# frgfm/Holocron

Measured on NVIDIA H100. Metric: images/sec RepVGG-A0 224^2 bf16 train, higher is better.
Workload: dtype bf16

## Files before the change

### holocron_b200/csrc/bn_act.cu

```cuda
#include <cstdio>
#include <cstdlib>
#include <type_traits>
#include <utility>
#include "common.cuh"
#include "act.cuh"
#include "slab.cuh"

namespace {

using namespace hb;

constexpr int kThreads = kSlabThreads;
constexpr int kMaxBranches = 3;

struct Branches {
  const __nv_bfloat16* u[kMaxBranches];
  int n;
};

__device__ __forceinline__ void fold_stat_partials(const SlabGeo& g, const float* red, int C, float* parts) {
  fold_row_lanes<double, 2>(g, red, [&](int c, const double (&a)[2]) {
    *reinterpret_cast<float2*>(parts + ((size_t)blockIdx.x * C + c) * 2) = make_float2((float)a[0], (float)a[1]);
  });
}
// ... 139 lines not shown
__global__ void bn_eval_affine_kernel(const float* gamma, const float* beta, const float* rmean, const float* rvar,
                                      float eps, int C, int C_logical, float* scale, float* shift, float* mean,
                                      float* rstd) {
  const int c = blockIdx.x * blockDim.x + threadIdx.x;
  if (c >= C) return;
  if (c >= C_logical) {
    scale[c] = 0.f; shift[c] = 0.f;
    if (mean) mean[c] = 0.f;
    if (rstd) rstd[c] = 0.f;
    return;
  }
  const float r = 1.f / sqrtf(rvar[c] + eps);
  const float sc = (gamma ? gamma[c] : 1.f) * r;
  scale[c] = sc;
  shift[c] = (beta ? beta[c] : 0.f) - rmean[c] * sc;
  if (mean) mean[c] = rmean[c];
  if (rstd) rstd[c] = r;
}

struct FwdParams {
  Branches br;
  const float* scale;
  const float* shift;
  const __nv_bfloat16* residual;
  __nv_bfloat16* out;
  int M, C, act;
  float slope;
  int res_after;
  float* out_stats;
};
using RawVec = Vec16<__nv_bfloat16>;

__device__ __forceinline__ void lds8(const float* p, float* f) {
  const float4 a = *reinterpret_cast<const float4*>(p);
  const float4 b = *reinterpret_cast<const float4*>(p + 4);
  f[0] = a.x; f[1] = a.y; f[2] = a.z; f[3] = a.w; f[4] = b.x; f[5] = b.y; f[6] = b.z; f[7] = b.w;
}

__host__ __device__ constexpr int ring_depth(int nt) { return nt <= 2 ? 7 : 3; }

__device__ __forceinline__ void cp_async16(uint32_t saddr, const void* g) {
  asm volatile("cp.async.cg.shared.global [%0], [%1], 16;" ::"r"(saddr), "l"(g) : "memory");
}
__device__ __forceinline__ void cp_async_commit() { asm volatile("cp.async.commit_group;" ::: "memory"); }
template <int N>
__device__ __forceinline__ void cp_async_wait() { asm volatile("cp.async.wait_group %0;" ::"n"(N) : "memory"); }
__device__ __forceinline__ RawVec lds16(uint32_t saddr) {
  RawVec r;
  asm volatile("ld.shared.v4.u32 {%0,%1,%2,%3}, [%4];" : "=r"(r.raw.x), "=r"(r.raw.y), "=r"(r.raw.z), "=r"(r.raw.w) : "r"(saddr));
  return r;
}
__device__ __forceinline__ uint32_t smem_addr(const void* p) { return (uint32_t)__cvta_generic_to_shared(p); }

template <int NT>
struct RowRing {
  static constexpr int kDepth = ring_depth(NT);
  static constexpr int kSlots = kDepth + 1;
  uint32_t base;
  size_t m0, stride, M;
  size_t col_off;
  int C;
  const __nv_bfloat16* src[NT > 0 ? NT : 1];
  __device__ __forceinline__ void init(uint8_t* smem, size_t m0_, size_t stride_, int M_, int C_, size_t col_off_) {
    base = smem_addr(smem) + threadIdx.x * 16;
    m0 = m0_; stride = stride_; M = (size_t)M_; col_off = col_off_; C = C_;
  }
  __device__ __forceinline__ uint32_t addr(int s, int t) const { return base + (uint32_t)((s * NT + t) * kThreads * 16); }
  __device__ __forceinline__ bool valid(size_t k) const { return m0 + k * stride < M; }
  __device__ __forceinline__ size_t off(size_t k) const { return (m0 + k * stride) * C + col_off; }
  __device__ __forceinline__ void issue(size_t k) const {
    if (valid(k)) {
      const int s = (int)(k % kSlots);
      const size_t o = off(k);
#pragma unroll
      for (int t = 0; t < NT; ++t)
        if (src[t]) cp_async16(addr(s, t), src[t] + o);
    }
    cp_async_commit();
  }
  __device__ __forceinline__ void prologue() const {
#pragma unroll
    for (int k = 0; k < kDepth; ++k) issue(k);
  }
  __device__ __forceinline__ void wait() const { cp_async_wait<kDepth - 1>(); }
};

template <int NB, bool kStats>
__global__ void __launch_bounds__(kThreads, 3) bn_act_fwd_kernel(FwdParams p, SlabGeo g) {
  extern __shared__ __align__(16) uint8_t ring_smem[];
  const auto [tx, ty, cg, active] = g.thread();
  float os[8], oq[8];
#pragma unroll
  for (int j = 0; j < 8; ++j) { os[j] = 0.f; oq[j] = 0.f; }
  __shared__ __align__(16) float k_sc[kMaxBranches][256];
  __shared__ __align__(16) float k_sh[256];
  {
    const int nch = g.cg_t * 8;
    for (int ch = threadIdx.x; ch < nch; ch += kThreads) {
      const int c = blockIdx.y * nch + ch;
      float shv = 0.f;
#pragma unroll
      for (int b = 0; b < NB; ++b) {
        k_sc[b][ch] = c < p.C ? p.scale[(size_t)b * p.C + c] : 0.f;
        shv += c < p.C ? p.shift[(size_t)b * p.C + c] : 0.f;
      }
      k_sh[ch] = shv;
    }
    __syncthreads();
  }
  if (!active && !kStats) return;
  if (active) {
    const bool has_res = p.residual != nullptr;
    RowRing<NB + 1> ring;
    ring.init(ring_smem, (size_t)blockIdx.x * g.rows_t + ty, (size_t)gridDim.x * g.rows_t, p.M, p.C, (size_t)cg * 8);
#pragma unroll
    for (int b = 0; b < NB; ++b) ring.src[b] = p.br.u[b];
    ring.src[NB] = p.residual;
    ring.prologue();
    for (size_t k = 0; ring.valid(k); ++k) {
      ring.wait();
      const int s = (int)(k % RowRing<NB + 1>::kSlots);
      RawVec u[NB > 0 ? NB : 1], r;
// ... 99 lines not shown
        const double mean = (double)p.mean[o], rstd = (double)p.rstd[o];
        const double mdzx = rstd * (p.sums[(size_t)(1 + b) * p.C + c] * invM - mean * mdz);
        const double cud = -(double)sc * rstd * mdzx;
        cu = (float)cud;
        c0 = (float)(-(double)sc * mdz - cud * mean);
      }
      k.cu[b][ch] = cu;
      k.c0[b][ch] = c0;
    }
    k.shift[ch] = sh;
  }
  __syncthreads();
}

template <int NB>
__device__ __forceinline__ void recompute_dz(const BwdParams& p, const SlabConsts& k, int ch0, const RawVec* uv,
                                             const RawVec& rv, const RawVec& dv, float (*u)[8], float* dz, float* dr) {
  float z[8];
  lds8(&k.shift[ch0], z);
#pragma unroll
  for (int b = 0; b < NB; ++b) {
    float sc[8];
    lds8(&k.scale[b][ch0], sc);
    unpack8(uv[b], u[b]);
#pragma unroll
    for (int j = 0; j < 8; ++j) z[j] = fmaf(sc[j], u[b][j], z[j]);
  }
  float d[8];
  unpack8(dv, d);
  if (p.residual && p.res_after) {
#pragma unroll
    for (int j = 0; j < 8; ++j) { dz[j] = d[j] * act_grad(p.act, z[j], p.slope); dr[j] = d[j]; }
    return;
  }
  if (p.residual) {
    float r[8];
    unpack8(rv, r);
    if (p.act == ACT_FRELU) {
#pragma unroll
      for (int j = 0; j < 8; ++j) {
        const float gate = z[j] > r[j] ? 1.f : (z[j] == r[j] ? 0.5f : 0.f);
        dz[j] = d[j] * gate;
        dr[j] = d[j] - dz[j];
      }
      return;
    }
#pragma unroll
    for (int j = 0; j < 8; ++j) z[j] += r[j];
  }
#pragma unroll
  for (int j = 0; j < 8; ++j) { dz[j] = d[j] * act_grad(p.act, z[j], p.slope); dr[j] = dz[j]; }
}

template <int NB>
__device__ __forceinline__ void init_bwd_ring(RowRing<NB + 2>& ring, const BwdParams& p, const SlabGeo& g, uint8_t* ring_smem,
                                              int ty, int cg) {
  ring.init(ring_smem, (size_t)blockIdx.x * g.rows_t + ty, (size_t)gridDim.x * g.rows_t, p.M, p.C, (size_t)cg * 8);
#pragma unroll
  for (int b = 0; b < NB; ++b) ring.src[b] = p.br.u[b];
  ring.src[NB] = (p.residual && !p.res_after) ? p.residual : nullptr;
  ring.src[NB + 1] = p.dout;
}

template <int NB>
__global__ void __launch_bounds__(kThreads, 2) bn_act_bwd_reduce_kernel(BwdParams p, SlabGeo g) {
  extern __shared__ __align__(16) uint8_t dyn_smem[];
  SlabConsts& k = *reinterpret_cast<SlabConsts*>(dyn_smem);
  float* red = reinterpret_cast<float*>(dyn_smem + sizeof(SlabConsts));
  uint8_t* ring_smem = dyn_smem + sizeof(SlabConsts) + kThreads * 8 * sizeof(float);
  load_slab_consts<NB>(k, p, g, false);
  const auto [tx, ty, cg, active] = g.thread();
  float acc[1 + NB][8];
#pragma unroll
  for (int i = 0; i < 1 + NB; ++i)
#pragma unroll
    for (int j = 0; j < 8; ++j) acc[i][j] = 0.f;
  if (active) {
    RowRing<NB + 2> ring;
    init_bwd_ring<NB>(ring, p, g, ring_smem, ty, cg);
    ring.prologue();
    for (size_t kk = 0; ring.valid(kk); ++kk) {
      ring.wait();
      const int s = (int)(kk % RowRing<NB + 2>::kSlots);
      RawVec uv[NB > 0 ? NB : 1], rv, dv;
#pragma unroll
      for (int b = 0; b < NB; ++b) uv[b] = lds16(ring.addr(s, b));
      if (ring.src[NB]) rv = lds16(ring.addr(s, NB));
      dv = lds16(ring.addr(s, NB + 1));
      ring.issue(kk + RowRing<NB + 2>::kDepth);
      float u[NB > 0 ? NB : 1][8], dz[8], dr[8];
      recompute_dz<NB>(p, k, tx * 8, uv, rv, dv, u, dz, dr);
#pragma unroll
      for (int j = 0; j < 8; ++j) acc[0][j] += dz[j];
#pragma unroll
      for (int b = 0; b < NB; ++b) {
#pragma unroll
        for (int j = 0; j < 8; ++j) acc[1 + b][j] = fmaf(dz[j], u[b][j], acc[1 + b][j]);
      }
    }
  }
#pragma unroll
  for (int i = 0; i < 1 + NB; ++i) {
    __syncthreads();
#pragma unroll
    for (int j = 0; j < 8; ++j) red[threadIdx.x * 8 + j] = acc[i][j];
    __syncthreads();
    fold_row_lanes<double, 1>(g, red, [&](int c, const double (&a)[1]) {
      p.part[((size_t)blockIdx.x * (1 + NB) + i) * p.C + c] = a[0];
    });
  }
}

template <int NB>
__global__ void __launch_bounds__(kThreads, 2) bn_act_bwd_apply_kernel(BwdParams p, SlabGeo g) {
  extern __shared__ __align__(16) uint8_t dyn_smem[];
  SlabConsts& k = *reinterpret_cast<SlabConsts*>(dyn_smem);
  uint8_t* ring_smem = dyn_smem + sizeof(SlabConsts);
  load_slab_consts<NB>(k, p, g, true);
  const auto [tx, ty, cg, active] = g.thread();
  if (!active) return;
  RowRing<NB + 2> ring;
  init_bwd_ring<NB>(ring, p, g, ring_smem, ty, cg);
  ring.prologue();
  for (size_t kk = 0; ring.valid(kk); ++kk) {
    ring.wait();
    const int s = (int)(kk % RowRing<NB + 2>::kSlots);
    RawVec uv[NB > 0 ? NB : 1], rv, dv;
#pragma unroll
    for (int b = 0; b < NB; ++b) uv[b] = lds16(ring.addr(s, b));
    if (ring.src[NB]) rv = lds16(ring.addr(s, NB));
    dv = lds16(ring.addr(s, NB + 1));
    ring.issue(kk + RowRing<NB + 2>::kDepth);
    const size_t off = ring.off(kk);
    float u[NB > 0 ? NB : 1][8], dz[8], dr[8];
    recompute_dz<NB>(p, k, tx * 8, uv, rv, dv, u, dz, dr);
    if (p.dres) store8(p.dres + off, dr);
#pragma unroll
    for (int b = 0; b < NB; ++b) {
      if (p.du[b]) {
        float sc[8], cu[8], c0[8], d[8];
        lds8(&k.scale[b][tx * 8], sc);
        lds8(&k.cu[b][tx * 8], cu);
        lds8(&k.c0[b][tx * 8], c0);
#pragma unroll
        for (int j = 0; j < 8; ++j) d[j] = fmaf(sc[j], dz[j], fmaf(cu[j], u[b][j], c0[j]));
        store8(p.du[b] + off, d);
      }
    }
  }
}

struct BwdFinalizeParams {
  const double* part; double* sums; const float* mean; const float* rstd;
  float* dgamma; float* dbeta;
  float* gacc[kMaxBranches]; float* bacc[kMaxBranches];
  int nblocks, B, C, C_logical;
};
__global__ void __launch_bounds__(kFinCh * kFinLanes) bn_bwd_finalize_kernel(BwdFinalizeParams p) {
  const int c = blockIdx.x * kFinCh + threadIdx.x;
  const size_t row = (size_t)(1 + p.B) * p.C;
  double tot[1 + kMaxBranches];
  fold_slots<1 + kMaxBranches>(c < p.C, p.nblocks, 1 + p.B, [&](int k, double (&v)[1 + kMaxBranches]) {
#pragma unroll
    for (int i = 0; i <= kMaxBranches; ++i)
      if (i <= p.B) v[i] = p.part[(size_t)k * row + (size_t)i * p.C + c];
  }, tot);
  if (threadIdx.y != 0 || c >= p.C) return;
  for (int i = 0; i <= p.B; ++i) p.sums[(size_t)i * p.C + c] = tot[i];
  for (int b = 0; b < p.B; ++b) {
    const size_t o = (size_t)b * p.C + c;
    const float dg = (float)((double)p.rstd[o] * (tot[1 + b] - (double)p.mean[o] * tot[0]));
    const float db = (float)tot[0];
    if (p.dgamma) p.dgamma[o] = dg;
    if (p.dbeta) p.dbeta[o] = db;
    if (c < p.C_logical) {
      if (p.gacc[b]) p.gacc[b][c] += dg;
      if (p.bacc[b]) p.bacc[b][c] += db;
    }
  }
}

inline dim3 make_grid(const SlabGeo& g, int M, int z, int per_sm = 4, int min_rows = 4) {
  long long row_blocks = ((long long)M + g.rows_t - 1) / g.rows_t;
  long long cap = (HB_NUM_SMS * per_sm) / g.slabs;
  if (cap < 1) cap = 1;
// ... 180 lines not shown
```

### holocron_b200/nn/_fused.py

```python
import ctypes
import functools
import os
import weakref
from typing import List, Optional, Sequence, Tuple

import torch
from torch import Tensor, nn

from .._lib import DTYPE_CODE, ConvArgs, check, dtype_code, lib, ptr, require_cuda, stream_ptr

ACT_NONE, ACT_RELU, ACT_RELU6, ACT_SILU, ACT_LEAKY, ACT_MISH, ACT_HARDMISH, ACT_FRELU = range(8)

_c_float = ctypes.c_float
_VP3 = ctypes.c_void_p * 3

KERNEL_TIMER = None


def _timed(kind: str, info: dict, fn):
    if KERNEL_TIMER is None:
        return fn()
    e0, e1 = torch.cuda.Event(enable_timing=True), torch.cuda.Event(enable_timing=True)
    e0.record()
    rc = fn()
# ... 244 lines not shown
    if v.numel() == n:
        return v
    out = torch.zeros(n, device=v.device, dtype=torch.float32)
    out[:v.numel()] = v
    return out


def conv_out_size(h: int, k: int, stride: int, pad: int, dil: int) -> int:
    return (h + 2 * pad - dil * (k - 1) - 1) // stride + 1


def conv2d_forward_raw(x: Tensor, wf: Tensor, cout: int, r: int, s: int, stride: int, pad: int, dil: int,
                       bias: Optional[Tensor] = None, residual: Optional[Tensor] = None, act: int = ACT_NONE, *,
                       w2: Optional[Tensor] = None, xe: Optional[Tensor] = None, we: Optional[Tensor] = None,
                       want_stats: bool = False, kind: str = "fprop", norm: Optional[Tuple[Tensor, Tensor, Tensor]] = None):
    n, cin_p, h, w = x.shape
    ho, wo = conv_out_size(h, r, stride, pad, dil), conv_out_size(w, s, stride, pad, dil)
    y = _empty_cl(n, cout, ho, wo, x.device)
    y2 = _empty_cl(n, cout, ho, wo, x.device) if w2 is not None else None
    a = ConvArgs()
    a.x, a.w, a.y = x.data_ptr(), wf.data_ptr(), y.data_ptr()
    a.bias = 0 if bias is None else bias.data_ptr()
    a.residual = 0 if residual is None else residual.data_ptr()
    a.N, a.H, a.W, a.Cin, a.Cout, a.R, a.S = n, h, w, cin_p, cout, r, s
    a.stride, a.pad, a.dil, a.act, a.num_ctas = stride, pad, dil, act, 0
    m_out = n * ho * wo
    k_total = r * s * cin_p
    in_elems = n * h * w * cin_p
    out_elems = m_out * cout
    w_elems = cout * r * s * cin_p
    if xe is not None:
        ce = xe.shape[1]
        a.xe, a.we, a.Ce = xe.data_ptr(), we.data_ptr(), ce
        k_total += ce
        in_elems += m_out * ce
        w_elems += cout * ce
    if w2 is not None:
        a.w2, a.y2 = w2.data_ptr(), y2.data_ptr()
        k_total += cin_p
        out_elems += m_out * cout
        w_elems += cout * cin_p
    if residual is not None:
        in_elems += m_out * cout
    if norm is not None:
        a.norm_mean, a.norm_rstd, a.norm_wsum = norm[0].data_ptr(), norm[1].data_ptr(), norm[2].data_ptr()
    st = st2 = None
    if want_stats:
        st = torch.empty((conv_stat_slots(x.device), cout, 2), device=x.device, dtype=torch.float32)
        a.stats = st.data_ptr()
        if w2 is not None:
            st2 = torch.empty((conv_stat_slots(x.device), cout, 2), device=x.device, dtype=torch.float32)
            a.stats2 = st2.data_ptr()
    slots = ctypes.c_int(0)
    info = dict(shape=(kind, h, cin_p, cout, r, stride), launches=1,
                **conv_work(m_out, cout, k_total, in_elems, w_elems, out_elems))
    check(_timed(kind, info, lambda: lib().hb_conv2d_fused_bf16(ctypes.byref(a), ctypes.byref(slots), stream_ptr())),
          "hb_conv2d_fused_bf16")
    if want_stats:
        if slots.value > st.shape[0]:
            raise RuntimeError("statistics slot capacity exceeded")
        attach_stats(y, st, slots.value)
        if y2 is not None:
            attach_stats(y2, st2, slots.value)
    return y if w2 is None else (y, y2)


class _Conv2dFn(torch.autograd.Function):

    @staticmethod
    def forward(ctx, x: Tensor, weight: Tensor, bias: Optional[Tensor], stride: int, pad: int, dil: int,
                keep_padded: bool, want_stats: bool = False) -> Tensor:
        cout, cin, r, s = weight.shape
        if x.shape[1] < cin:
            raise RuntimeError(f"expected an input with at least {cin} channels, got {x.shape[1]}")
        need_dx = ctx.needs_input_grad[0]
        if (cin <= 4 and x.shape[1] == cin and r == 3 and s == 3 and pad == 1 and dil == 1 and not need_dx and x.is_contiguous()
                and x.dtype in DTYPE_CODE and cout % 16 == 0 and not os.environ.get("HB_DISABLE_STEM_IM2COL")):
            col, wp, _ = _stem_im2col(x, weight, stride)
            y = conv2d_forward_raw(col, wp, cout, 1, 1, 1, 0, 1, _pad_vec(bias, cout),
                                   want_stats=want_stats and epilogue_stats_pay_off(col.shape[1]))
            ctx.save_for_backward(col, weight)
            ctx.cfg = ("stem", bias is not None)
            return y
        y, pk, xb = _packed_conv(x, weight, bias, stride, pad, dil, need_dgrad=need_dx, keep_padded=keep_padded,
                                 want_stats=want_stats)
        ctx.save_for_backward(xb, weight)
        ctx.cfg = (stride, pad, dil, pk.wd, bias is not None, x.shape[1], pk.cout_p, pk.cin_d)
        return y

    @staticmethod
    def backward(ctx, dy: Tensor):
        xb, weight = ctx.saved_tensors
        if ctx.cfg[0] == "stem":
            cout = weight.shape[0]
            dyb = to_channels_last_bf16(dy, cout)
            dw = db = None
            if ctx.needs_input_grad[1]:
                dw = _stem_wgrad(xb, dyb, weight)
            if ctx.cfg[1] and ctx.needs_input_grad[2]:
                db = dyb.float().sum((0, 2, 3))
            return None, dw, db, None, None, None, None, None
        stride, pad, dil, wd, has_bias, cin_x, cout_p, cin_d = ctx.cfg
        cout = weight.shape[0]
        h, w = xb.shape[2], xb.shape[3]
        dyb = to_channels_last_bf16(dy, cout_p)
        dx = dw = db = None
        if ctx.needs_input_grad[0]:
# ... 85 lines not shown
def _wgrad(xb: Tensor, dyb: Tensor, weight: Tensor, stride: int, pad: int, dil: int = 1) -> Optional[Tensor]:
    cout, cin, r, s = weight.shape
    if r != s:
        raise NotImplementedError("non-square filters")
    cout_p, cin_p = dyb.shape[1], xb.shape[1]
    g = direct_grad(weight, krsc=True) if (cin_p == cin and cout_p == cout) else None
    if g is not None and wgrad_raw(xb, dyb, cout_p, r, stride, pad, dil, acc_into=g) is None:
        return None
    return _wgrad_to_param(wgrad_raw(xb, dyb, cout_p, r, stride, pad, dil), weight)


def conv2d_bias_act(x: Tensor, weight: Tensor, bias: Optional[Tensor], stride: int, padding: int, act: int = ACT_NONE,
                    slope: float = 0.0) -> Tensor:
    require_cuda(x, weight)
    needs_grad = torch.is_grad_enabled() and (x.requires_grad or weight.requires_grad or
                                              (bias is not None and bias.requires_grad))
    if not needs_grad and act in (ACT_NONE, ACT_RELU):
        return _packed_conv(x, weight, bias, stride, padding, 1, act)[0]
    if act == ACT_NONE:
        return _Conv2dFn.apply(x, weight, bias, int(stride), int(padding), 1, False, False)
    y = act_only(_Conv2dFn.apply(x, weight, bias, int(stride), int(padding), 1, True, False), act, slope)
    return y if y.shape[1] == weight.shape[0] else y[:, :weight.shape[0]]


class BNBranch:
    __slots__ = ("running_mean", "running_var", "eps", "momentum", "num_batches_tracked", "track_running_stats")

    def __init__(self, bn: nn.BatchNorm2d) -> None:
        self.running_mean = bn.running_mean
        self.running_var = bn.running_var
        self.eps = bn.eps
        self.momentum = bn.momentum
        self.num_batches_tracked = bn.num_batches_tracked
        self.track_running_stats = bn.track_running_stats and bn.running_mean is not None


def _arr3(ts: Sequence[Optional[Tensor]]):
    vals = [0 if t is None else t.data_ptr() for t in ts]
    return _VP3(*(vals + [0] * (3 - len(vals))))


_I3 = ctypes.c_int * 3


def _elem_bytes_info(kind: str, m: int, c: int, reads: int, writes: int) -> dict:
    return dict(shape=(kind, m, c, reads, writes), launches=1, flops=0.0, bytes=2.0 * m * c * (reads + writes))


def _bn_batch_stats(us: Sequence[Tensor], branches, g32, b32, stats: Tensor, c: int, c_log: int, m: int) -> None:
    if m == 1:
        raise ValueError(f"Expected more than 1 value per channel when training, got input size {us[0].shape}")
    L = lib()
    nb = len(us)
    parts, slots = [], []
    for u in us:
        st = get_stats(u)
        if st is None:
            buf = torch.empty((bn_stat_slots(u.device), c, 2), device=u.device, dtype=torch.float32)
            sl = ctypes.c_int(0)
            check(_timed("bn_stats", _elem_bytes_info("bn_stats", m, c, 1, 0), lambda: L.hb_bn_stats_partials_bf16(
                ptr(u), m, c, ptr(buf), ctypes.byref(sl), stream_ptr())), "hb_bn_stats_partials_bf16")
            st = (buf, sl.value)
        parts.append(st[0])
        slots.append(st[1])
    eps, mom = branches[0].eps, branches[0].momentum
    if any(b.eps != eps or b.momentum != mom for b in branches):
        raise NotImplementedError("branches with different eps/momentum")
    track = [b.track_running_stats for b in branches]
    if mom is None and any(track):
        raise NotImplementedError("cumulative moving average (momentum=None)")
    check(L.hb_bn_finalize(_arr3(parts), _I3(*(slots + [0] * (3 - nb))), _arr3(g32), _arr3(b32),
                           _arr3([b.running_mean if t else None for b, t in zip(branches, track)]),
                           _arr3([b.running_var if t else None for b, t in zip(branches, track)]),
                           _arr3([b.num_batches_tracked if t else None for b, t in zip(branches, track)]),
                           ptr(stats[0]), ptr(stats[1]), ptr(stats[2]), ptr(stats[3]), nb, c, c_log, m, _c_float(eps),
                           _c_float(0.0 if mom is None else mom), stream_ptr()), "hb_bn_finalize")


def _bn_forward_pass(us: Sequence[Tensor], stats: Tensor, res: Optional[Tensor], m: int, c: int, act: int, slope: float,
                     res_after: int, shape, emit_stats: bool) -> Tensor:
    n, _, h, w = shape
    nb = len(us)
    dev = us[0].device if nb else res.device
    if emit_stats and os.environ.get("HB_DISABLE_BN_OUT_STATS"):
        emit_stats = False
    out = _empty_cl(n, c, h, w, dev)
    ost = torch.empty((bn_stat_slots(dev), c, 2), device=dev, dtype=torch.float32) if emit_stats else None
    sl = ctypes.c_int(0)
    up = [ptr(us[i]) if i < nb else ptr(None) for i in range(3)]
    check(_timed("bn_fwd", _elem_bytes_info("bn_fwd", m, c, nb + (res is not None), 1), lambda: lib().hb_bn_act_fwd_bf16(
        up[0], up[1], up[2], nb, ptr(stats[2]), ptr(stats[3]), ptr(res), ptr(out), m, c, act, _c_float(slope), int(res_after),
        ptr(ost), ctypes.byref(sl) if emit_stats else None, stream_ptr())), "hb_bn_act_fwd_bf16")
    if emit_stats:
        attach_stats(out, ost, sl.value)
    return out


def _bn_backward_pass(dob: Tensor, us: Sequence[Tensor], stats: Tensor, res: Optional[Tensor], dus, dres, dgb, gacc, bacc,
                      c_log: int, m: int, c: int, act: int, slope: float, training: bool, res_after: int) -> None:
    L = lib()
    nb = len(us)
    scratch = torch.empty(L.hb_bn_bwd_scratch_doubles(m, c, nb), device=dob.device, dtype=torch.float64)
    up = [ptr(us[i]) if i < nb else ptr(None) for i in range(3)]
    dup = [ptr(dus[i]) if i < nb else ptr(None) for i in range(3)]
    nres = int(res is not None and not res_after)
    nwr = sum(d is not None for d in dus) + (dres is not None)
    info = _elem_bytes_info("bn_bwd", m, c, 2 * (1 + nb + nres), nwr)
    info["launches"] = 3
    check(_timed("bn_bwd", info, lambda: L.hb_bn_act_bwd_bf16(
        ptr(dob), up[0], up[1], up[2], nb, ptr(stats[2]), ptr(stats[3]), ptr(stats[0]), ptr(stats[1]), ptr(res), ptr(scratch),
        dup[0], dup[1], dup[2], ptr(dres), ptr(dgb[0]) if dgb is not None else ptr(None),
        ptr(dgb[1]) if dgb is not None else ptr(None), _arr3(gacc) if gacc is not None else None,
        _arr3(bacc) if bacc is not None else None, c_log, m, c, act, _c_float(slope), 1 if training else 0, res_after,
        stream_ptr())), "hb_bn_act_bwd_bf16")


def _bn_setup(us: Sequence[Tensor], branches, gammas: Sequence[Tensor], betas: Sequence[Tensor], training: bool, c: int,
# ... 66 lines not shown
        grads += dus
        grads += [dgb[0][i][:c_log] if dgb is not None else None for i in range(nb)]
        grads += [dgb[1][i][:c_log] if dgb is not None else None for i in range(nb)]
        if has_res:
            grads.append(dres)
        return tuple(grads)


def bn_act(us: Sequence[Tensor], bns: Sequence[nn.BatchNorm2d], act: int = ACT_NONE, slope: float = 0.0,
           residual: Optional[Tensor] = None, training: Optional[bool] = None, res_after_act: bool = False,
           emit_stats: bool = False) -> Tensor:
    if not 1 <= len(us) <= 3 or len(us) != len(bns):
        raise ValueError("between 1 and 3 (input, BatchNorm2d) pairs are supported")
    require_cuda(*us)
    if training is None:
        training = bns[0].training
    use_batch_stats = training or bns[0].running_mean is None
    cfg = ([BNBranch(b) for b in bns], int(act), float(slope), bool(use_batch_stats), residual is not None,
           bool(res_after_act), bool(emit_stats))
    args = list(us) + [b.weight for b in bns] + [b.bias for b in bns]
    if residual is not None:
        args.append(residual)
    return _BNActFn.apply(cfg, *args)


def act_only(x: Tensor, act: int, slope: float = 0.0) -> Tensor:
    cfg = ([], int(act), float(slope), False, True, False, False)
    return _BNActFn.apply(cfg, x)


class _RepBlockFn(torch.autograd.Function):

    @staticmethod
    def forward(ctx, cfg, x: Tensor, w3: Tensor, w1: Tensor, *bn_params: Tensor) -> Tensor:
        branches, act, slope, training, stride = cfg
        nb = len(branches)
        gammas, betas = bn_params[:nb], bn_params[nb:]
        need_dx = ctx.needs_input_grad[1]
        cout, cin = w3.shape[0], w3.shape[1]
        if cout % 16 != 0:
            raise NotImplementedError("fused RepBlock needs out_channels % 16 == 0")
        stem = cin <= 4 and x.shape[1] == cin and not need_dx and x.is_contiguous() and x.dtype in DTYPE_CODE
        if stem:
            xb, wf3, wf1 = _stem_im2col(x, w3, stride, w1)
            k3, conv_stride, pad3 = 1, 1, 0
            wd3 = wd1 = None
        else:
            pk3 = pack_filter(w3, need_dx, round_up(x.shape[1], 8))
            pk1 = pack_filter(w1, need_dx, round_up(x.shape[1], 8))
            xb = to_channels_last_bf16(x, pk3.cin_p)
            wf3, wf1, wd3, wd1 = pk3.wf, pk1.wf, pk3.wd, pk1.wd
            k3, conv_stride, pad3 = 3, stride, 1
        kx = xb.shape[1]
        if os.environ.get("HB_FUSED_FPROP"):
            y3, y1 = conv2d_forward_raw(xb, wf3, cout, k3, k3, conv_stride, pad3, 1, w2=wf1,
                                        want_stats=training and epilogue_stats_pay_off(k3 * k3 * kx))
        else:
            y3 = conv2d_forward_raw(xb, wf3, cout, k3, k3, conv_stride, pad3, 1,
                                    want_stats=training and epilogue_stats_pay_off(k3 * k3 * kx))
            y1 = conv2d_forward_raw(xb, wf1, cout, 1, 1, conv_stride, 0, 1,
                                    want_stats=training and epilogue_stats_pay_off(kx))
        us = [y3, y1] + ([xb] if nb == 3 else [])
        n, c, h, w = y3.shape
        m = n * h * w
        stats = _bn_setup(us, branches, gammas, betas, training, c, c, m, y3.device)
        out = _bn_forward_pass(us, stats, None, m, c, act, slope, 0, (n, c, h, w), emit_stats=training)
        ctx.save_for_backward(stats, xb, y3, y1, w3, w1, *gammas, *betas)
        ctx.cfg = (nb, act, slope, training, stride, wd3, wd1, x.shape[1], stem)
        return out

    @staticmethod
    def backward(ctx, dout: Tensor):
        nb, act, slope, training, stride, wd3, wd1, cin_x, stem = ctx.cfg
        stats, xb, y3, y1, w3, w1 = ctx.saved_tensors[:6]
        gammas, betas = ctx.saved_tensors[6:6 + nb], ctx.saved_tensors[6 + nb:6 + 2 * nb]
        n, c, ho, wo = y3.shape
        _, cin_p, h, w = xb.shape
        m = n * ho * wo
        dev = dout.device
        L = lib()
        dob = to_channels_last_bf16(dout)
        need_dx = ctx.needs_input_grad[1]
        dy3, dy1 = _empty_cl(n, c, ho, wo, dev), _empty_cl(n, c, ho, wo, dev)
        dxid = _empty_cl(n, c, ho, wo, dev) if (nb == 3 and need_dx) else None
        gacc, bacc, dgb = _bn_grad_targets(gammas, betas, c, dev)
        us = [y3, y1] + ([xb] if nb == 3 else [])
        _bn_backward_pass(dob, us, stats, None, [dy3, dy1] + ([dxid] if nb == 3 else []), None, dgb, gacc, bacc, c, m, c, act,
                          slope, training, 0)
        g_gamma = [None if dgb is None else dgb[0][i] for i in range(nb)]
        g_beta = [None if dgb is None else dgb[1][i] for i in range(nb)]
        dx = None
        if need_dx:
            cin_d = wd3.shape[0]
            if stride == 1 and wd3.shape[3] == c and (dxid is None or cin_d == c):
                dxp = None
                if not os.environ.get("HB_DISABLE_CONV_ROWS"):
                    eye = _identity_filter(cin_d, c, dev) if dxid is not None else None
                    dxr = _empty_cl(n, cin_d, h, w, dev)
                    nsrc = 2 if dxid is not None else 1
                    info = dict(shape=("dgrad_rows", h, c, cin_d, 3, 1), launches=1,
                                **conv_work(n * h * w, cin_d, 10 * c, (1 + nsrc) * n * h * w * c, 10 * cin_d * c))
                    rc = _timed("dgrad", info, lambda: L.hb_conv3x3_accum_bf16(
                        ptr(dy3), ptr(wd3), ptr(dy1), ptr(wd1), ptr(dxid), ptr(eye), nsrc, ptr(dxr), n, h, w, c, cin_d, 0,
                        stream_ptr()))
                    if rc == 0:
                        dxp = dxr
                    elif rc != 801:
                        check(rc, "hb_conv3x3_accum_bf16")
                if dxp is None:
                    dxp = conv2d_forward_raw(dy3, wd3, cin_d, 3, 3, 1, 1, 1, None, dxid, ACT_NONE, xe=dy1, we=wd1, kind="dgrad")
            else:
                dxp = _dgrad(dy3, w3, wd3, cin_d, h, w, stride, 1, dy1, wd1)
# ... 144 lines not shown
```

### holocron_b200/csrc/conv_wgrad.cu

```cuda
#include <cstdlib>
#include "conv_common.cuh"

namespace {

using namespace tc;
using namespace conv;

constexpr int kBKpix = 64;
constexpr int kChunkBytes = kBKpix * 128;
constexpr int kABytes = 2 * kChunkBytes;

struct WgradParams {
  int m_total, Ho, Wo, stride, pad, dil, R, S, Cin, Cout;
  int ci_tile;
  int ci_chunks;
  int taps_per_group;
  int num_tap_groups, num_co_tiles, num_ci_tiles, k_splits;
  int kblocks_total;
  int stages, stage_bytes;
  int use_atomics;
  float* dw;
  float* ws;
  long long dw_elems;
};

template <int CIW>
__global__ void __launch_bounds__(kThreads, 1)
conv_wgrad_kernel(const __grid_constant__ CUtensorMap tmDY, const __grid_constant__ CUtensorMap tmX, const WgradParams p) {
  constexpr int kChunks = (CIW + 63) / 64, kNLast = CIW - 64 * (kChunks - 1);
  extern __shared__ __align__(1024) uint8_t smem_raw[];
  uint8_t* smem = reinterpret_cast<uint8_t*>((reinterpret_cast<uintptr_t>(smem_raw) + 1023) & ~uintptr_t(1023));
  uint64_t* full_bar = reinterpret_cast<uint64_t*>(smem + (size_t)p.stages * p.stage_bytes);
  uint64_t* empty_bar = full_bar + p.stages;

  const int warp = threadIdx.x >> 5, lane = threadIdx.x & 31;
  if (warp == 0 && lane == 0) {
    prefetch_tmap(&tmDY);
    prefetch_tmap(&tmX);
    for (int i = 0; i < p.stages; ++i) { mbar_init(&full_bar[i], 1); mbar_init(&empty_bar[i], kConsumers / 32); }
    fence_barrier_init();
  }
  __syncthreads();

  const int RS = p.R * p.S;
  const int num_units = p.num_co_tiles * p.num_ci_tiles * p.num_tap_groups * p.k_splits;
  const int b_tap_bytes = p.ci_chunks * kChunkBytes;

  auto decode = [&](int unit, int& co_t, int& ci_t, int& tg, int& ks) {
    ks = unit % p.k_splits; unit /= p.k_splits;
    tg = unit % p.num_tap_groups; unit /= p.num_tap_groups;
    ci_t = unit % p.num_ci_tiles; co_t = unit / p.num_ci_tiles;
  };
  auto kb_range = [&](int ks, int& kb0, int& kb1) {
    const int per = (p.kblocks_total + p.k_splits - 1) / p.k_splits;
    kb0 = ks * per;
    kb1 = min(kb0 + per, p.kblocks_total);
  };

  if (warp < 4) {
    if (warp == 0 && lane == 0) {
      Ring ring;
      for (int unit = blockIdx.x; unit < num_units; unit += gridDim.x) {
        int co_t, ci_t, tg, ks, kb0, kb1;
        decode(unit, co_t, ci_t, tg, ks);
        kb_range(ks, kb0, kb1);
        const int tap0 = tg * p.taps_per_group;
        const int ntaps = min(p.taps_per_group, RS - tap0);
        const uint32_t tx = kABytes + ntaps * b_tap_bytes;
        for (int kb = kb0; kb < kb1; ++kb) {
          const int m0 = kb * kBKpix;
          const int q0 = m0 % p.Wo, p0 = (m0 / p.Wo) % p.Ho, n0 = m0 / (p.Wo * p.Ho);
          const int base_w = q0 * p.stride - p.pad, base_h = p0 * p.stride - p.pad;
          uint64_t* bar = &full_bar[ring.stage];
          mbar_wait(&empty_bar[ring.stage], ring.phase ^ 1);
          uint8_t* sa = smem + (size_t)ring.stage * p.stage_bytes;
          mbar_arrive_expect_tx(bar, tx);
          tma_load_2d(&tmDY, bar, sa, co_t * 128, m0);
          tma_load_2d(&tmDY, bar, sa + kChunkBytes, co_t * 128 + 64, m0);
          for (int t = 0; t < ntaps; ++t) {
            const int tap = tap0 + t, r = tap / p.S, s = tap % p.S;
            uint8_t* sb = sa + kABytes + t * b_tap_bytes;
            for (int c = 0; c < p.ci_chunks; ++c)
              tma_load_im2col_4d(&tmX, bar, sb + c * kChunkBytes, ci_t * p.ci_tile + c * 64, base_w, base_h, n0,
                                 (uint16_t)(s * p.dil), (uint16_t)(r * p.dil));
          }
          ring.next(p.stages);
        }
      }
    }
    return;
  }

  const int et = threadIdx.x - 128;
  const int wg = et >> 7;
  const int frow = frag_row(et & 127), fcol = frag_col(et & 127);
  const uint32_t dhi = desc_hi(1024);
  float acc[CIW / 2];
  Ring ring;
  for (int unit = blockIdx.x; unit < num_units; unit += gridDim.x) {
    int co_t, ci_t, tg, ks, kb0, kb1;
    decode(unit, co_t, ci_t, tg, ks);
    kb_range(ks, kb0, kb1);
    const int tap = tg * p.taps_per_group;
    int prev = -1;
    for (int kb = kb0; kb < kb1; ++kb) {
      mbar_wait(&full_bar[ring.stage], ring.phase);
      const uint32_t s_lo = desc_lo(smem_u32(smem + (size_t)ring.stage * p.stage_bytes), 16);
      const uint32_t a_lo = s_lo + (uint32_t)wg * (kChunkBytes >> 4);
      const uint32_t b_lo = s_lo + (kABytes >> 4);
      const uint32_t acc0 = kb > kb0 ? 1u : 0u;
      wgmma_fence();
#pragma unroll
      for (int k = 0; k < kBKpix / 16; ++k) {
        const uint64_t ad = make_desc(a_lo + k * (2048 >> 4), dhi);
        const uint32_t sc = acc0 | (uint32_t)k;
        if constexpr (kChunks == 1) {
          wgmma<kNLast, 1, 1>(acc, ad, make_desc(b_lo + k * (2048 >> 4), dhi), sc);
        } else {
          wgmma<64, 1, 1>(acc, ad, make_desc(b_lo + k * (2048 >> 4), dhi), sc);
          wgmma<kNLast, 1, 1>(acc + 32, ad, make_desc(b_lo + (kChunkBytes >> 4) + k * (2048 >> 4), dhi), sc);
        }
      }
      wgmma_commit();
      wgmma_wait<1>();
      if (prev >= 0 && lane == 0) mbar_arrive(&empty_bar[prev]);
      prev = ring.stage;
      ring.next(p.stages);
    }
    wgmma_wait<0>();
    fence_regs(acc);
    if (prev >= 0 && lane == 0) mbar_arrive(&empty_bar[prev]);

    const bool have = kb1 > kb0;
    if (!have && p.use_atomics != 2) continue;
    float* base = p.use_atomics == 2 ? p.ws + (size_t)ks * p.dw_elems : p.dw;
#pragma unroll
    for (int h = 0; h < 2; ++h) {
      const int co = co_t * 128 + 64 * wg + frow + 8 * h;
      if (co >= p.Cout) continue;
      float* drow = base + ((size_t)co * RS + tap) * p.Cin;
#pragma unroll
      for (int j = 0; j < CIW / 8; ++j) {
        const int c = (j >> 3) * 64 + 8 * (j & 7) + fcol;
        const int ci = ci_t * p.ci_tile + c;
        if (c >= p.ci_tile || ci >= p.Cin) continue;
        const float v0 = have ? acc[4 * j + 2 * h] : 0.f, v1 = have ? acc[4 * j + 2 * h + 1] : 0.f;
        if (p.use_atomics == 1) {
          atomicAdd(drow + ci, v0);
          atomicAdd(drow + ci + 1, v1);
        } else {
          *reinterpret_cast<float2*>(drow + ci) = make_float2(v0, v1);
        }
      }
    }
  }
}

__global__ void __launch_bounds__(256) wgrad_reduce_kernel(const float* __restrict__ ws, float* __restrict__ dw, long long n,
                                                           int k_splits, float* __restrict__ dw2, long long n_first,
                                                           int accumulate) {
  __shared__ float4 part[8][32];
  const long long i4 = ((long long)blockIdx.x * 32 + threadIdx.x) * 4;
  const int y = threadIdx.y;
  float4 acc = make_float4(0.f, 0.f, 0.f, 0.f);
  if (i4 + 3 < n) {
#pragma unroll 4
    for (int k = y; k < k_splits; k += 8) {
      const float4 v = *reinterpret_cast<const float4*>(ws + (size_t)k * n + i4);
      acc.x += v.x; acc.y += v.y; acc.z += v.z; acc.w += v.w;
    }
  } else if (i4 < n) {
    float t[4] = {0.f, 0.f, 0.f, 0.f};
    for (int k = y; k < k_splits; k += 8)
      for (int j = 0; j < 4 && i4 + j < n; ++j) t[j] += ws[(size_t)k * n + i4 + j];
    acc = make_float4(t[0], t[1], t[2], t[3]);
  }
  part[y][threadIdx.x] = acc;
  __syncthreads();
  if (y == 0 && i4 < n) {
    float4 r = part[0][threadIdx.x];
#pragma unroll
    for (int j = 1; j < 8; ++j) {
      const float4 v = part[j][threadIdx.x];
      r.x += v.x; r.y += v.y; r.z += v.z; r.w += v.w;
    }
    float* dst = i4 < n_first ? dw + i4 : dw2 + (i4 - n_first);
    if (i4 + 3 < n) {
      if (accumulate) {
        const float4 o = *reinterpret_cast<const float4*>(dst);
        r.x += o.x; r.y += o.y; r.z += o.z; r.w += o.w;
      }
      *reinterpret_cast<float4*>(dst) = r;
    } else {
      const float t[4] = {r.x, r.y, r.z, r.w};
      for (int j = 0; j < 4 && i4 + j < n; ++j) dst[j] = accumulate ? dst[j] + t[j] : t[j];
    }
  }
}

inline void launch_wgrad_reduce(const float* ws, float* dw, long long n, int slices, cudaStream_t st, float* dw2 = nullptr,
                                long long n_first = -1, int accumulate = 0) {
  const unsigned blocks = (unsigned)((n / 4 + 32) / 32);
  if (n_first < 0 || !dw2) { n_first = n; dw2 = dw; }
  wgrad_reduce_kernel<<<blocks, dim3(32, 8), 0, st>>>(ws, dw, n, slices, dw2, n_first, accumulate);
}

struct WgradPlan {
  WgradParams p;
  size_t ws_bytes;
};

int plan_wgrad(WgradPlan& plan, int N, int H, int W, int Cin, int Cout, int R, int S, int stride, int pad, int dil,
               int num_ctas) {
  WgradParams& p = plan.p;
  const int Ho = (H + 2 * pad - dil * (R - 1) - 1) / stride + 1;
  const int Wo = (W + 2 * pad - dil * (S - 1) - 1) / stride + 1;
  const long long m_ll = (long long)N * Ho * Wo;
  if (Ho <= 0 || Wo <= 0 || m_ll > 0x7fffffffLL) return (int)cudaErrorInvalidValue;
  p.m_total = (int)m_ll; p.Ho = Ho; p.Wo = Wo; p.stride = stride; p.pad = pad; p.dil = dil;
  p.R = R; p.S = S; p.Cin = Cin; p.Cout = Cout;
  const int RS = R * S;
  int ci_tile = Cin;
  if (Cin > 128) {
    ci_tile = 128;
    if (Cin % 128 != 0 && Cin % 64 == 0) ci_tile = 64;
  }
  p.ci_tile = ci_tile;
  p.ci_chunks = (ci_tile + 63) / 64;
  p.taps_per_group = 1;
  p.stage_bytes = kABytes + p.ci_chunks * kChunkBytes;
  p.stages = (200 * 1024) / p.stage_bytes;
  if (p.stages > 6) p.stages = 6;
  p.num_tap_groups = (RS + p.taps_per_group - 1) / p.taps_per_group;
  p.num_co_tiles = (Cout + 127) / 128;
  p.num_ci_tiles = (Cin + ci_tile - 1) / ci_tile;
  p.kblocks_total = (p.m_total + kBKpix - 1) / kBKpix;
  const int base_units = p.num_co_tiles * p.num_ci_tiles * p.num_tap_groups;
  const int ctas = num_ctas > 0 ? num_ctas : HB_NUM_SMS;
  int k_splits = (2 * ctas + base_units - 1) / base_units;
  if (base_units >= ctas) k_splits = 1;
  const int max_splits = (p.kblocks_total + 7) / 8;
  if (k_splits > max_splits) k_splits = max_splits;
  if (k_splits < 1) k_splits = 1;
  p.k_splits = k_splits;
  p.dw_elems = (long long)Cout * RS * Cin;
  plan.ws_bytes = k_splits > 1 ? (size_t)k_splits * p.dw_elems * sizeof(float) : 0;
  return 0;
}

}

extern "C" {

size_t hb_conv2d_wgrad_workspace_bytes(int N, int H, int W, int Cin, int Cout, int R, int S, int stride, int pad, int dil,
                                       int num_ctas) {
  WgradPlan plan{};
  if (plan_wgrad(plan, N, H, W, Cin, Cout, R, S, stride, pad, dil, num_ctas)) return 0;
  const size_t rows = hb_wgrad_rows_workspace_bytes(N, H, W, Cin, Cout, R, S, stride, pad, dil, num_ctas, 0);
  return rows > plan.ws_bytes ? rows : plan.ws_bytes;
}

static int wgrad_impl(const void* x, const void* dy, float* dw, float* workspace, size_t workspace_bytes, int N, int H,
                      int W, int Cin, int Cout, int R, int S, int stride, int pad, int dil, int num_ctas, void* stream,
                      int accumulate) {
  if (Cin % 8 != 0 || Cout % 8 != 0) return (int)cudaErrorInvalidValue;
  if (!hb::aligned16(x) || !hb::aligned16(dy) || !hb::aligned16(dw)) return (int)cudaErrorMisalignedAddress;
  cudaStream_t st = (cudaStream_t)stream;
  static const bool rows_enabled = getenv("HB_DISABLE_WGRAD_ROWS") == nullptr;
  if (rows_enabled && R == 3 && S == 3 && stride == 1 && pad == 1 && dil == 1 && workspace && hb::aligned16(workspace)) {
    int slices = 0;
    const int rc = hb_wgrad_rows_try(x, dy, nullptr, workspace, workspace_bytes, N, H, W, Cin, Cout, num_ctas, st, &slices);
    if (rc == 0) {
      const long long n = (long long)Cout * 9 * Cin;
      launch_wgrad_reduce(workspace, dw, n, slices, st, nullptr, -1, accumulate);
      HB_LAUNCH_CHECK();
      return 0;
    }
    if (rc != (int)cudaErrorNotSupported) return rc;
  }
  WgradPlan plan{};
  if (int rc = plan_wgrad(plan, N, H, W, Cin, Cout, R, S, stride, pad, dil, num_ctas)) return rc;
  WgradParams& p = plan.p;
  if (accumulate && !(p.k_splits > 1 && workspace && workspace_bytes >= plan.ws_bytes && hb::aligned16(workspace)))
    return (int)cudaErrorNotSupported;
  const int RS = R * S;
  const int k_splits = p.k_splits;
  const int base_units = p.num_co_tiles * p.num_ci_tiles * p.num_tap_groups;
  const int ctas = num_ctas > 0 ? num_ctas : HB_NUM_SMS;
  p.dw = dw;
  p.ws = workspace;
  if (k_splits == 1) {
    p.use_atomics = 0;
  } else if (workspace && workspace_bytes >= plan.ws_bytes && hb::aligned16(workspace)) {
    p.use_atomics = 2;
  } else {
    p.use_atomics = 1;
    cudaError_t e = cudaMemsetAsync(dw, 0, (size_t)Cout * RS * Cin * sizeof(float), st);
    if (e != cudaSuccess) return (int)e;
  }

  CUtensorMap tmDY, tmX;
  if (int rc = tmap::encode_matrix(&tmDY, dy, p.m_total, Cout, kBKpix)) return rc;
  if (int rc = tmap::encode_im2col_bf16(&tmX, x, N, H, W, Cin, pad, pad, R, S, dil, stride, 64, kBKpix,
                                        CU_TENSOR_MAP_SWIZZLE_128B))
    return rc;
  const size_t smem_bytes = (size_t)p.stages * p.stage_bytes + 2 * p.stages * sizeof(uint64_t) + 1024;
  const int num_units = base_units * k_splits;
  int grid = ctas < num_units ? ctas : num_units;
  const cudaError_t e = dispatch_width<16, 128>((p.ci_tile + 15) & ~15, [&](auto ciw) {
    return launch<conv_wgrad_kernel<decltype(ciw)::value>>(grid, smem_bytes, st, tmDY, tmX, p);
  });
  if (e != cudaSuccess) return (int)e;
  if (p.use_atomics == 2) {
    const long long n = p.dw_elems;
    launch_wgrad_reduce(workspace, dw, n, k_splits, st, nullptr, -1, accumulate);
    HB_LAUNCH_CHECK();
  }
  return 0;
}

int hb_conv2d_wgrad_bf16(const void* x, const void* dy, float* dw, float* workspace, size_t workspace_bytes, int N, int H,
                         int W, int Cin, int Cout, int R, int S, int stride, int pad, int dil, int num_ctas, void* stream) {
  return wgrad_impl(x, dy, dw, workspace, workspace_bytes, N, H, W, Cin, Cout, R, S, stride, pad, dil, num_ctas, stream, 0);
}

int hb_conv2d_wgrad_acc_bf16(const void* x, const void* dy, float* dw, float* workspace, size_t workspace_bytes, int N, int H,
                             int W, int Cin, int Cout, int R, int S, int stride, int pad, int dil, int num_ctas,
                             void* stream) {
  return wgrad_impl(x, dy, dw, workspace, workspace_bytes, N, H, W, Cin, Cout, R, S, stride, pad, dil, num_ctas, stream, 1);
}

size_t hb_repvgg_wgrad_workspace_bytes(int N, int H, int W, int Cin, int Cout, int num_ctas) {
  return hb_wgrad_rows_workspace_bytes(N, H, W, Cin, Cout, 3, 3, 1, 1, 1, num_ctas, 1);
}

static int repvgg_wgrad_impl(const void* x, const void* dy3, const void* dy1, float* dw, float* dw1, float* workspace,
                             size_t workspace_bytes, int N, int H, int W, int Cin, int Cout, int num_ctas, void* stream,
                             int accumulate) {
  if (Cin % 8 != 0 || Cout % 8 != 0) return (int)cudaErrorInvalidValue;
  if (!hb::aligned16(x) || !hb::aligned16(dy3) || !hb::aligned16(dy1) || !hb::aligned16(dw) || !hb::aligned16(workspace) ||
      !hb::aligned16(dw1))
    return (int)cudaErrorMisalignedAddress;
  cudaStream_t st = (cudaStream_t)stream;
  int slices = 0;
  if (int rc = hb_wgrad_rows_try(x, dy3, dy1, workspace, workspace_bytes, N, H, W, Cin, Cout, num_ctas, st, &slices))
// ... 20 lines not shown
```

Before: 9258.

## Reverse bwd-apply row order, reorder BN stats, fuse stem 3x3+1x1 fprop

The backward apply kernel now walks its rows in reverse order, so the tail just touched by the reduce pass is read first while it may still sit in L2. Per-branch BN stats are now computed last-to-first so the most recently produced tensor is scanned first. The stem block always uses the fused dual-output forward conv instead of two separate launches. Row iteration is now counted by a precomputed row count, not a bounds compare.

```diff
diff --git a/holocron_b200/csrc/bn_act.cu b/holocron_b200/csrc/bn_act.cu
--- a/holocron_b200/csrc/bn_act.cu
+++ b/holocron_b200/csrc/bn_act.cu
@@ -215,22 +215,23 @@
 }
 __device__ __forceinline__ uint32_t smem_addr(const void* p) { return (uint32_t)__cvta_generic_to_shared(p); }
 
-template <int NT>
+template <int NT, bool kReverse = false>
 struct RowRing {
   static constexpr int kDepth = ring_depth(NT);
   static constexpr int kSlots = kDepth + 1;
   uint32_t base;
-  size_t m0, stride, M;
+  size_t m0, stride, rows;
   size_t col_off;
   int C;
   const __nv_bfloat16* src[NT > 0 ? NT : 1];
   __device__ __forceinline__ void init(uint8_t* smem, size_t m0_, size_t stride_, int M_, int C_, size_t col_off_) {
     base = smem_addr(smem) + threadIdx.x * 16;
-    m0 = m0_; stride = stride_; M = (size_t)M_; col_off = col_off_; C = C_;
+    m0 = m0_; stride = stride_; col_off = col_off_; C = C_;
+    rows = m0_ < (size_t)M_ ? ((size_t)M_ - m0_ + stride_ - 1) / stride_ : 0;
   }
   __device__ __forceinline__ uint32_t addr(int s, int t) const { return base + (uint32_t)((s * NT + t) * kThreads * 16); }
-  __device__ __forceinline__ bool valid(size_t k) const { return m0 + k * stride < M; }
-  __device__ __forceinline__ size_t off(size_t k) const { return (m0 + k * stride) * C + col_off; }
+  __device__ __forceinline__ bool valid(size_t k) const { return k < rows; }
+  __device__ __forceinline__ size_t off(size_t k) const { return (m0 + (kReverse ? rows - 1 - k : k) * stride) * C + col_off; }
   __device__ __forceinline__ void issue(size_t k) const {
     if (valid(k)) {
       const int s = (int)(k % kSlots);
@@ -436,9 +437,9 @@
   for (int j = 0; j < 8; ++j) { dz[j] = d[j] * act_grad(p.act, z[j], p.slope); dr[j] = dz[j]; }
 }
 
-template <int NB>
-__device__ __forceinline__ void init_bwd_ring(RowRing<NB + 2>& ring, const BwdParams& p, const SlabGeo& g, uint8_t* ring_smem,
-                                              int ty, int cg) {
+template <int NB, bool kReverse>
+__device__ __forceinline__ void init_bwd_ring(RowRing<NB + 2, kReverse>& ring, const BwdParams& p, const SlabGeo& g,
+                                              uint8_t* ring_smem, int ty, int cg) {
   ring.init(ring_smem, (size_t)blockIdx.x * g.rows_t + ty, (size_t)gridDim.x * g.rows_t, p.M, p.C, (size_t)cg * 8);
 #pragma unroll
   for (int b = 0; b < NB; ++b) ring.src[b] = p.br.u[b];
@@ -503,18 +504,19 @@
   load_slab_consts<NB>(k, p, g, true);
   const auto [tx, ty, cg, active] = g.thread();
   if (!active) return;
-  RowRing<NB + 2> ring;
+  using Ring = RowRing<NB + 2, true>;
+  Ring ring;
   init_bwd_ring<NB>(ring, p, g, ring_smem, ty, cg);
   ring.prologue();
   for (size_t kk = 0; ring.valid(kk); ++kk) {
     ring.wait();
-    const int s = (int)(kk % RowRing<NB + 2>::kSlots);
+    const int s = (int)(kk % Ring::kSlots);
     RawVec uv[NB > 0 ? NB : 1], rv, dv;
 #pragma unroll
     for (int b = 0; b < NB; ++b) uv[b] = lds16(ring.addr(s, b));
     if (ring.src[NB]) rv = lds16(ring.addr(s, NB));
     dv = lds16(ring.addr(s, NB + 1));
-    ring.issue(kk + RowRing<NB + 2>::kDepth);
+    ring.issue(kk + Ring::kDepth);
     const size_t off = ring.off(kk);
     float u[NB > 0 ? NB : 1][8], dz[8], dr[8];
     recompute_dz<NB>(p, k, tx * 8, uv, rv, dv, u, dz, dr);
diff --git a/holocron_b200/nn/_fused.py b/holocron_b200/nn/_fused.py
--- a/holocron_b200/nn/_fused.py
+++ b/holocron_b200/nn/_fused.py
@@ -320,7 +320,7 @@
             st2 = torch.empty((conv_stat_slots(x.device), cout, 2), device=x.device, dtype=torch.float32)
             a.stats2 = st2.data_ptr()
     slots = ctypes.c_int(0)
-    info = dict(shape=(kind, h, cin_p, cout, r, stride), launches=1,
+    info = dict(shape=(kind, h, cin_p, cout, r, stride), launches=1, stats=want_stats,
                 **conv_work(m_out, cout, k_total, in_elems, w_elems, out_elems))
     check(_timed(kind, info, lambda: lib().hb_conv2d_fused_bf16(ctypes.byref(a), ctypes.byref(slots), stream_ptr())),
           "hb_conv2d_fused_bf16")
@@ -512,8 +512,9 @@
         raise ValueError(f"Expected more than 1 value per channel when training, got input size {us[0].shape}")
     L = lib()
     nb = len(us)
-    parts, slots = [], []
-    for u in us:
+    parts, slots = [None] * nb, [0] * nb
+    for i in reversed(range(nb)):
+        u = us[i]
         st = get_stats(u)
         if st is None:
             buf = torch.empty((bn_stat_slots(u.device), c, 2), device=u.device, dtype=torch.float32)
@@ -521,8 +522,7 @@
             check(_timed("bn_stats", _elem_bytes_info("bn_stats", m, c, 1, 0), lambda: L.hb_bn_stats_partials_bf16(
                 ptr(u), m, c, ptr(buf), ctypes.byref(sl), stream_ptr())), "hb_bn_stats_partials_bf16")
             st = (buf, sl.value)
-        parts.append(st[0])
-        slots.append(st[1])
+        parts[i], slots[i] = st
     eps, mom = branches[0].eps, branches[0].momentum
     if any(b.eps != eps or b.momentum != mom for b in branches):
         raise NotImplementedError("branches with different eps/momentum")
@@ -695,12 +695,11 @@
             wf3, wf1, wd3, wd1 = pk3.wf, pk1.wf, pk3.wd, pk1.wd
             k3, conv_stride, pad3 = 3, stride, 1
         kx = xb.shape[1]
-        if os.environ.get("HB_FUSED_FPROP"):
-            y3, y1 = conv2d_forward_raw(xb, wf3, cout, k3, k3, conv_stride, pad3, 1, w2=wf1,
-                                        want_stats=training and epilogue_stats_pay_off(k3 * k3 * kx))
+        stats3 = training and epilogue_stats_pay_off(k3 * k3 * kx)
+        if stem or os.environ.get("HB_FUSED_FPROP"):
+            y3, y1 = conv2d_forward_raw(xb, wf3, cout, k3, k3, conv_stride, pad3, 1, w2=wf1, want_stats=stats3)
         else:
-            y3 = conv2d_forward_raw(xb, wf3, cout, k3, k3, conv_stride, pad3, 1,
-                                    want_stats=training and epilogue_stats_pay_off(k3 * k3 * kx))
+            y3 = conv2d_forward_raw(xb, wf3, cout, k3, k3, conv_stride, pad3, 1, want_stats=stats3)
             y1 = conv2d_forward_raw(xb, wf1, cout, 1, 1, conv_stride, 0, 1,
                                     want_stats=training and epilogue_stats_pay_off(kx))
         us = [y3, y1] + ([xb] if nb == 3 else [])
```

New measurement: 9321, median of 6. Within noise of the previous version (+0.7%).

## Pair two filter taps per CTA in wgrad when Cout fits one half-tile

Applied to the files above, without the earlier changes.

For Cout <= 64, each CTA now handles two filter taps instead of one. Each consumer warpgroup computes one tap against the shared dY tile, and the second dY half-load is skipped when it would be entirely out of bounds. The k-split count is still computed from the full tap count, and a new accumulate mode (read-add-write) lets the single-split path handle accumulate instead of returning not-supported. This targets wasted MMA work and the redundant dY loads for narrow layers, at the cost of larger stages and therefore fewer pipeline stages.

```diff
diff --git a/holocron_b200/csrc/conv_wgrad.cu b/holocron_b200/csrc/conv_wgrad.cu
--- a/holocron_b200/csrc/conv_wgrad.cu
+++ b/holocron_b200/csrc/conv_wgrad.cu
@@ -66,7 +66,8 @@
         kb_range(ks, kb0, kb1);
         const int tap0 = tg * p.taps_per_group;
         const int ntaps = min(p.taps_per_group, RS - tap0);
-        const uint32_t tx = kABytes + ntaps * b_tap_bytes;
+        const bool box1 = p.taps_per_group == 1 && co_t * 128 + 64 < p.Cout;
+        const uint32_t tx = (box1 ? kABytes : kChunkBytes) + ntaps * b_tap_bytes;
         for (int kb = kb0; kb < kb1; ++kb) {
           const int m0 = kb * kBKpix;
           const int q0 = m0 % p.Wo, p0 = (m0 / p.Wo) % p.Ho, n0 = m0 / (p.Wo * p.Ho);
@@ -76,7 +77,7 @@
           uint8_t* sa = smem + (size_t)ring.stage * p.stage_bytes;
           mbar_arrive_expect_tx(bar, tx);
           tma_load_2d(&tmDY, bar, sa, co_t * 128, m0);
-          tma_load_2d(&tmDY, bar, sa + kChunkBytes, co_t * 128 + 64, m0);
+          if (box1) tma_load_2d(&tmDY, bar, sa + kChunkBytes, co_t * 128 + 64, m0);
           for (int t = 0; t < ntaps; ++t) {
             const int tap = tap0 + t, r = tap / p.S, s = tap % p.S;
             uint8_t* sb = sa + kABytes + t * b_tap_bytes;
@@ -93,6 +94,9 @@
 
   const int et = threadIdx.x - 128;
   const int wg = et >> 7;
+  const bool pairs = p.taps_per_group == 2;
+  const int wtap = pairs ? wg : 0;
+  const int wco = pairs ? 0 : 64 * wg;
   const int frow = frag_row(et & 127), fcol = frag_col(et & 127);
   const uint32_t dhi = desc_hi(1024);
   float acc[CIW / 2];
@@ -101,13 +105,13 @@
     int co_t, ci_t, tg, ks, kb0, kb1;
     decode(unit, co_t, ci_t, tg, ks);
     kb_range(ks, kb0, kb1);
-    const int tap = tg * p.taps_per_group;
+    const int tap = tg * p.taps_per_group + wtap;
     int prev = -1;
     for (int kb = kb0; kb < kb1; ++kb) {
       mbar_wait(&full_bar[ring.stage], ring.phase);
       const uint32_t s_lo = desc_lo(smem_u32(smem + (size_t)ring.stage * p.stage_bytes), 16);
-      const uint32_t a_lo = s_lo + (uint32_t)wg * (kChunkBytes >> 4);
-      const uint32_t b_lo = s_lo + (kABytes >> 4);
+      const uint32_t a_lo = s_lo + (uint32_t)wco * (128 >> 4);
+      const uint32_t b_lo = s_lo + ((kABytes + wtap * b_tap_bytes) >> 4);
       const uint32_t acc0 = kb > kb0 ? 1u : 0u;
       wgmma_fence();
 #pragma unroll
@@ -132,11 +136,28 @@
     if (prev >= 0 && lane == 0) mbar_arrive(&empty_bar[prev]);
 
     const bool have = kb1 > kb0;
-    if (!have && p.use_atomics != 2) continue;
+    if ((!have && p.use_atomics != 2) || tap >= RS) continue;
     float* base = p.use_atomics == 2 ? p.ws + (size_t)ks * p.dw_elems : p.dw;
+    if (p.use_atomics == 3) {
+#pragma unroll
+      for (int h = 0; h < 2; ++h) {
+        const int co = co_t * 128 + wco + frow + 8 * h;
+        if (co >= p.Cout) continue;
+        const float* drow = base + ((size_t)co * RS + tap) * p.Cin;
+#pragma unroll
+        for (int j = 0; j < CIW / 8; ++j) {
+          const int c = (j >> 3) * 64 + 8 * (j & 7) + fcol;
+          const int ci = ci_t * p.ci_tile + c;
+          if (c >= p.ci_tile || ci >= p.Cin) continue;
+          const float2 o = *reinterpret_cast<const float2*>(drow + ci);
+          acc[4 * j + 2 * h] = o.x + acc[4 * j + 2 * h];
+          acc[4 * j + 2 * h + 1] = o.y + acc[4 * j + 2 * h + 1];
+        }
+      }
+    }
 #pragma unroll
     for (int h = 0; h < 2; ++h) {
-      const int co = co_t * 128 + 64 * wg + frow + 8 * h;
+      const int co = co_t * 128 + wco + frow + 8 * h;
       if (co >= p.Cout) continue;
       float* drow = base + ((size_t)co * RS + tap) * p.Cin;
 #pragma unroll
@@ -227,15 +248,15 @@
   }
   p.ci_tile = ci_tile;
   p.ci_chunks = (ci_tile + 63) / 64;
-  p.taps_per_group = 1;
-  p.stage_bytes = kABytes + p.ci_chunks * kChunkBytes;
+  p.taps_per_group = Cout <= 64 && RS > 1 ? 2 : 1;
+  p.stage_bytes = kABytes + p.taps_per_group * p.ci_chunks * kChunkBytes;
   p.stages = (200 * 1024) / p.stage_bytes;
   if (p.stages > 6) p.stages = 6;
   p.num_tap_groups = (RS + p.taps_per_group - 1) / p.taps_per_group;
   p.num_co_tiles = (Cout + 127) / 128;
   p.num_ci_tiles = (Cin + ci_tile - 1) / ci_tile;
   p.kblocks_total = (p.m_total + kBKpix - 1) / kBKpix;
-  const int base_units = p.num_co_tiles * p.num_ci_tiles * p.num_tap_groups;
+  const int base_units = p.num_co_tiles * p.num_ci_tiles * RS;
   const int ctas = num_ctas > 0 ? num_ctas : HB_NUM_SMS;
   int k_splits = (2 * ctas + base_units - 1) / base_units;
   if (base_units >= ctas) k_splits = 1;
@@ -281,7 +302,7 @@
   WgradPlan plan{};
   if (int rc = plan_wgrad(plan, N, H, W, Cin, Cout, R, S, stride, pad, dil, num_ctas)) return rc;
   WgradParams& p = plan.p;
-  if (accumulate && !(p.k_splits > 1 && workspace && workspace_bytes >= plan.ws_bytes && hb::aligned16(workspace)))
+  if (accumulate && p.k_splits > 1 && !(workspace && workspace_bytes >= plan.ws_bytes && hb::aligned16(workspace)))
     return (int)cudaErrorNotSupported;
   const int RS = R * S;
   const int k_splits = p.k_splits;
@@ -290,7 +311,7 @@
   p.dw = dw;
   p.ws = workspace;
   if (k_splits == 1) {
-    p.use_atomics = 0;
+    p.use_atomics = accumulate ? 3 : 0;
   } else if (workspace && workspace_bytes >= plan.ws_bytes && hb::aligned16(workspace)) {
     p.use_atomics = 2;
   } else {
```

After: 9268 before, 9434 after (median of 6 runs). 1.02x the previous value.
